# jacarvalho/mpd-public

Measured on AMD Instinct MI355X. Metric: denoising-steps/s, higher is better.
Workload: dtype f32; 1 GPU; cfg2: EnvDense2D-RobotPointMass shape, 100 trajectories (1 context(s)) x H=64 x D=4, T=100 (+5) reverse steps, unguided, U-Net dim_mults (1, 2, 4, 8), one plan = one bench step; parallelism=single, denoising_steps_per_plan=105

## Files before the change

### include/mpdx.h

```cpp
#ifndef MPDX_H
#define MPDX_H

#include <stddef.h>
#include <stdint.h>

#ifdef __cplusplus
extern "C" {
#endif

#define MPDX_E_INVALID   (-1)
#define MPDX_E_NOTFOUND  (-2)
#define MPDX_E_STATE     (-3)

#define MPDX_MAX_LEVELS 8

typedef struct mpdx_unet mpdx_unet;

typedef struct mpdx_unet_cfg {
    int32_t state_dim;
    int32_t n_support_points;
    int32_t unet_input_dim;
    int32_t n_levels;
    int32_t dim_mults[MPDX_MAX_LEVELS];
    int32_t time_emb_dim;
    int32_t self_attention;
} mpdx_unet_cfg;

const char* mpdx_last_error(void);
int mpdx_version(void);

int    mpdx_unet_create(const mpdx_unet_cfg* cfg, mpdx_unet** out);
void   mpdx_unet_destroy(mpdx_unet* u);
int    mpdx_unet_set_plan_join(mpdx_unet* u, int on);
int    mpdx_unet_plan_joined(const mpdx_unet* u);
int    mpdx_unet_num_params(const mpdx_unet* u);
int    mpdx_unet_param_info(const mpdx_unet* u, int idx, const char** name, int32_t shape[3], int32_t* ndim);
size_t mpdx_unet_packed_floats(const mpdx_unet* u);
size_t mpdx_unet_timetab_floats(const mpdx_unet* u, int T);
size_t mpdx_unet_workspace_floats(const mpdx_unet* u, int B);
int    mpdx_unet_pack_param(mpdx_unet* u, const char* name, const float* src_dev, size_t n_floats,
                            float* packed_dev, void* stream);
int    mpdx_unet_build_timetab(mpdx_unet* u, const float* packed_dev, const float* freqs16_dev, int T,
                               float* timetab_dev, void* stream);

int mpdx_unet_forward(mpdx_unet* u, const float* packed_dev, const float* timetab_dev, int T,
                      const float* x, int t, float* eps, int B, float* ws, void* stream);

typedef struct mpdx_step_coefs {
    float sqrt_recip_alphas_cumprod;
// ... 198 lines not shown
```

### mpd_public_amd/_lib.py

```python
from __future__ import annotations

import ctypes as C
from pathlib import Path

import os as _os

_LIB_PATH = Path(_os.environ["MPDX_LIB"]) if _os.environ.get("MPDX_LIB") else Path(__file__).resolve().parent / "libmpdx.so"
_lib = None

MAX_LEVELS = 8


class UnetCfg(C.Structure):
    _fields_ = [("state_dim", C.c_int32), ("n_support_points", C.c_int32), ("unet_input_dim", C.c_int32),
                ("n_levels", C.c_int32), ("dim_mults", C.c_int32 * MAX_LEVELS), ("time_emb_dim", C.c_int32),
                ("self_attention", C.c_int32)]


class StepCoefs(C.Structure):
    _fields_ = [("sqrt_recip_alphas_cumprod", C.c_float), ("sqrt_recipm1_alphas_cumprod", C.c_float),
                ("posterior_mean_coef1", C.c_float), ("posterior_mean_coef2", C.c_float),
                ("noise_scale", C.c_float), ("noise_std_extra", C.c_float),
                ("predict_epsilon", C.c_int32), ("clip_denoised", C.c_int32), ("ddim_k1", C.c_float), ("ddim_k2", C.c_float),
                ("guide_scale", C.c_float)]
# ... 41 lines not shown

class IkOpts(C.Structure):
    _fields_ = [("frame", C.c_int32), ("offset", C.c_float * 3), ("q_lo", C.c_float * 8), ("q_hi", C.c_float * 8), ("rot_weight", C.c_float),
                ("pos_tol", C.c_float), ("rot_tol", C.c_float), ("lambda_init", C.c_float), ("lambda_up", C.c_float), ("lambda_down", C.c_float),
                ("lambda_min", C.c_float), ("lambda_max", C.c_float), ("adaptive", C.c_int32), ("max_iters", C.c_int32), ("seed", C.c_uint64)]


_vp, _sz, _i, _f = C.c_void_p, C.c_size_t, C.c_int, C.c_float
SIGNATURES = {
    "mpdx_last_error": (C.c_char_p, []),
    "mpdx_version": (_i, []),
    "mpdx_unet_create": (_i, [C.POINTER(UnetCfg), C.POINTER(_vp)]),
    "mpdx_unet_destroy": (None, [_vp]),
    "mpdx_unet_set_plan_join": (_i, [_vp, _i]),
    "mpdx_unet_plan_joined": (_i, [_vp]),
    "mpdx_unet_num_params": (_i, [_vp]),
    "mpdx_unet_param_info": (_i, [_vp, _i, C.POINTER(C.c_char_p), C.POINTER(C.c_int32 * 3), C.POINTER(C.c_int32)]),
    "mpdx_unet_packed_floats": (_sz, [_vp]),
    "mpdx_unet_timetab_floats": (_sz, [_vp, _i]),
    "mpdx_unet_workspace_floats": (_sz, [_vp, _i]),
    "mpdx_unet_pack_param": (_i, [_vp, C.c_char_p, _vp, _sz, _vp, _vp]),
    "mpdx_unet_build_timetab": (_i, [_vp, _vp, _vp, _i, _vp, _vp]),
    "mpdx_unet_forward": (_i, [_vp, _vp, _vp, _i, _vp, _i, _vp, _i, _vp, _vp]),
    "mpdx_ddpm_step": (_i, [_vp, _vp, _vp, _i, _vp, _vp, _vp, _vp, C.POINTER(StepCoefs), _i, _i, _vp, _vp, _i, _i, _vp, _vp]),
    "mpdx_add_noise": (_i, [_vp, _vp, _vp, _vp, _f, _f, _vp, _i, _i, _i, _vp]),
    "mpdx_hard_conds": (_i, [_vp, _vp, _i, C.POINTER(C.c_int32), C.POINTER(_vp), _i, _i, _i, _vp]),
    "mpdx_q_sample": (_i, [_vp, _vp, _vp, _vp, _vp, _vp, _vp, _vp, _i, _i, _i, _i, _vp]),
    "mpdx_weighted_loss": (_i, [_vp, _vp, _vp, _vp, _vp, _i, _vp, _i, _i, _i, _vp]),
    "mpdx_plan": (_i, [_vp, _vp, _vp, _i, C.POINTER(StepCoefs), _i, _vp, _vp, _vp, _vp, _vp, _i, _vp,
                        C.POINTER(GuideParams), _i, _i, _vp, _i, C.c_uint64, C.c_uint64, _vp]),
# ... 83 lines not shown
```

### mpd_public_amd/csrc/conv_block.hpp

```cpp
#pragma once
#include <hip/hip_runtime.h>
#include <stdint.h>

#include <type_traits>

#if defined(MPDX_LOOP_ABLATION) && !defined(MPDX_DEV_HOOKS)
#define MPDX_DEV_HOOKS 1
#endif
#ifdef MPDX_DEV_HOOKS
#define MPDX_TRACE_PTR(p) (p)
#define MPDX_DBG(a, bits) ((a).dbg & (bits))
#else
#define MPDX_TRACE_PTR(p) ((long long*)nullptr)
#define MPDX_DBG(a, bits) (0)
#endif

namespace mpdx {

typedef float f32x4 __attribute__((ext_vector_type(4)));
typedef float f32x2 __attribute__((ext_vector_type(2)));

enum : int { CONV_S1 = 0, CONV_DOWN = 1, CONV_UPT = 2 };
enum : int { EPI_BIAS = 0, EPI_GN_MISH = 1, EPI_GN_MISH_GEN = 2, EPI_GN_BWD = 3 };

// ... 127 lines not shown

template <int MODE, int KS>
struct ConvGeom {
    static constexpr int PAD = (MODE == CONV_S1) ? KS / 2 : 1;
    static constexpr int NTAP = (MODE == CONV_UPT) ? 2 : KS;
    static constexpr int NSLOT = (MODE == CONV_UPT) ? 4 : KS;
};

__host__ __device__ inline int upt_slot_to_k(int slot) { return slot == 0 ? 1 : slot == 1 ? 3 : slot == 2 ? 2 : 0; }

struct GeoAny { static constexpr int L = 0, NC16 = 0, RSPAD = 0; };
template <int NC16_> struct GeoL8 { static constexpr int L = 8, NC16 = NC16_, RSPAD = 8; };
template <int NC16_> struct GeoUp8 { static constexpr int L = 8, NC16 = NC16_, RSPAD = 4; };
constexpr int geo_ilog2(int v) { return v <= 1 ? 0 : 1 + geo_ilog2(v >> 1); }

template <int MODE, int KS, int EPI, int MT, int NT, int WN, int WK, class GEO = GeoAny, int TBRES = -1>
__device__ __forceinline__ void conv_block_body(const ConvArgs& a, const int block_id) {
    using G = ConvGeom<MODE, KS>;
    constexpr bool GK = GEO::L > 0;
    static_assert(!GK || MODE == CONV_S1 || MODE == CONV_UPT, "compile-time geometry: stride-1 and transposed convolutions on 8 input positions");
    constexpr int NWAVE = WN * WK, NTHR = 64 * NWAVE;
    constexpr int MS = MT / 16, NSUB = NT / 16, NSW = NSUB / WN;
    constexpr int PAD = G::PAD, NTAP = G::NTAP, NSLOT = G::NSLOT;
    constexpr int MTP = MT + 4;
    constexpr int MTP4 = MTP / 4;
    static_assert(NSUB % WN == 0, "N split");
    static_assert(MODE != CONV_UPT || (NSW % 2 == 0), "transposed conv pairs even/odd sub-tiles");

    extern __shared__ __attribute__((aligned(16))) float smem[];

    const int tid = threadIdx.x, lane = tid & 63;
    if constexpr (GK) __builtin_assume(tid < NTHR);
// ... 33 lines not shown
#pragma unroll
            for (int p = 0; p < NCLS; ++p) {
                const int slot = (MODE == CONV_UPT) ? (p * 2 + ts) : ts;
                dst[m][p] = __builtin_bit_cast(f32x4, __builtin_amdgcn_raw_buffer_load_b128(wrs, wlane, wtile + ((m * nc16 + c16) * NSLOT + slot) * 1024, 0));
            }
    };
    const int niter = (ngroups + WK - 1) / WK;
    auto ring_g = [&](int it) { const int g = wk + it * WK; return g < ngroups ? g : ngroups - 1; };
    auto ring_init = [&]() {
#pragma unroll
        for (int u = 0; u < PF; ++u) load_a(ring_g(u), af[u]);
    };
#ifdef MPDX_RING_FIRST
    ring_init();
#endif

    if (!MPDX_DBG(a, 1)) {
        const int total = (spt << lg_Lin) << lg_c4n;
        const bool vec_ok = GK ? true : ((a.c1 & 3) == 0) && ((a.c2 & 3) == 0);
        constexpr int SB = 4;
        auto stage_pass = [&](int base, auto vec, auto first) {
            constexpr bool VEC = decltype(vec)::value;
            constexpr bool FIRST = decltype(first)::value;
            f32x4 v[SB];
            int dsto[SB], cc[SB];
            bool ok[SB];
            size_t pos[SB];
#pragma unroll
            for (int u = 0; u < SB; ++u) {
                const int idx = base + u * NTHR;
                const bool in = idx < total;
                const int idc = in ? idx : 0;
                const int rowi = idc >> lg_c4n, c = (idc & (c4n - 1)) << 2;
                const int s = rowi >> lg_Lin, li = rowi & (L_in - 1);
                const int b = s0 + s;
                dsto[u] = in ? (s * LP + li + PAD) * RS4 + (c >> 2) : -1;
                ok[u] = in && b < a.B && c < cin;
                cc[u] = c < cin ? c : 0;
                pos[u] = (size_t)(b < a.B ? b : a.B - 1) * L_in + li;
                if (a.stuff) { ok[u] = ok[u] && !(li & 1); pos[u] = (size_t)(b < a.B ? b : a.B - 1) * (L_in >> 1) + (li >> 1); }
            }
#pragma unroll
            for (int u = 0; u < SB; ++u) {
                if constexpr (VEC) {
                    const float* src = (cc[u] < a.c1) ? a.src1 + pos[u] * a.c1 + cc[u] : a.src2 + pos[u] * a.c2 + (cc[u] - a.c1);
                    v[u] = *(const f32x4*)src;
                } else {
#pragma unroll
                    for (int e = 0; e < 4; ++e) {
                        const int ce = cc[u] + e;
                        const float* src = (ce < a.c1) ? a.src1 + pos[u] * a.c1 + ce : (ce < cin) ? a.src2 + pos[u] * a.c2 + (ce - a.c1) : a.src1 + pos[u] * a.c1;
                        v[u][e] = *src;
                    }
                }
            }
#ifndef MPDX_RING_FIRST
            if constexpr (FIRST) ring_init();
#endif
#pragma unroll
            for (int u = 0; u < SB; ++u) {
                if constexpr (!VEC) {
#pragma unroll
                    for (int e = 0; e < 4; ++e) v[u][e] = (cc[u] + e < cin) ? v[u][e] : 0.f;
                }
                if (dsto[u] >= 0) smem4[dsto[u]] = ok[u] ? v[u] : (f32x4){0.f, 0.f, 0.f, 0.f};
            }
        };
        if (vec_ok) {
            stage_pass(tid, std::true_type{}, std::true_type{});
            for (int base = tid + NTHR * SB; base < total; base += NTHR * SB) stage_pass(base, std::true_type{}, std::false_type{});
        } else {
            stage_pass(tid, std::false_type{}, std::true_type{});
            for (int base = tid + NTHR * SB; base < total; base += NTHR * SB) stage_pass(base, std::false_type{}, std::false_type{});
        }
        if (PAD > 0) {
            constexpr int P2 = PAD > 0 ? 2 * PAD : 1;
            const int htot = (spt * P2) << lg_c4n;
            for (int idx = tid; idx < htot; idx += NTHR) {
                const int hr = idx >> lg_c4n, c4 = idx & (c4n - 1);
                const int s = hr / P2, k = hr - s * P2;
                const int lp = (k < PAD) ? k : (L_in + k);
                smem4[(s * LP + lp) * RS4 + c4] = (f32x4){0.f, 0.f, 0.f, 0.f};
            }
        }
    }
#ifndef MPDX_RING_FIRST
    if (MPDX_DBG(a, 1)) ring_init();
#endif
    CB_STAMP();
    __syncthreads();
    CB_STAMP();

    const int j = lane & 15, q = lane >> 4;
    int boff[NSW];
    int npos[NSW];
#pragma unroll
    for (int i = 0; i < NSW; ++i) {
        const int ns = wn * NSW + i;
        if (MODE == CONV_UPT) {
            const int gm = (ns >> 1) * 16 + j;
            const int s = gm >> lg_Lin, m = gm & (L_in - 1);
            boff[i] = (s * LP + m + PAD) * RS4 + q;
// ... 58 lines not shown

    CB_STAMP();
    __syncthreads();
    CB_STAMP();
    float* red = smem;
#pragma unroll
    for (int m = 0; m < MS; ++m)
#pragma unroll
        for (int i = 0; i < NSW; ++i)
            smem4[(wk * NT + npos[i]) * MTP4 + m * 4 + q] = acc[m][i];
    __syncthreads();
    CB_STAMP();

    if (MPDX_DBG(a, 4)) {
        if (tid == 0 && red[0] == 123.456f) a.dst[0] = red[1];
        return;
    }
    if constexpr (EPI == EPI_GN_MISH_GEN) {
        const int gs = a.gs;
        const int lg_gpt = (MT == 32 ? 5 : 4) - a.lg_gs;
        const int gpt = 1 << lg_gpt;
        const int nreg = spt << lg_gpt;
        const int re = gs << a.lg_Lout;
        const int Lv = (a.Lv_out > 0 && a.Lv_out < L_out) ? a.Lv_out : L_out;
        const float inv_re = 1.0f / (float)(gs * Lv);
        auto region = [&](auto w_, auto nch_, int s, int gl, int b) {
            constexpr int W = decltype(w_)::value, NCH = decltype(nch_)::value;
            float v[NCH][W], tb[NCH][W], rsd[NCH][W], ga[NCH][W], be[NCH][W];
            size_t o[NCH];
            bool ok[NCH];
            float sum = 0.f;
// ... 140 lines not shown
            if (re == 256) region(std::integral_constant<int, 4>{}, s, gl, s0 + s);
            else region(std::integral_constant<int, 2>{}, s, gl, s0 + s);
        }
    } else
    if (EPI == EPI_GN_MISH) {
        const int gs = a.gs;
        const int lg_gpt = (MT == 32 ? 5 : 4) - a.lg_gs;
        const int gpt = 1 << lg_gpt;
        const int nreg = spt << lg_gpt;
        const int re = gs << lg_Lout;
        const bool has_tb = TBRES < 0 ? a.tbias != nullptr : TBRES == 1, has_res = TBRES < 0 ? a.res != nullptr : TBRES == 2;
        const float inv_re = (re == 256) ? (1.0f / 256.0f) : (1.0f / 128.0f);
        for (int r = wave; r < nreg; r += NWAVE) {
            const int s = r >> lg_gpt, gl = r & (gpt - 1);
            const int b = s0 + s;
            if (re == 256) {
                const int e0 = lane * 4;
                const int l = e0 >> a.lg_gs, c = gl * gs + (e0 & (gs - 1));
                const int n = s * L_out + l, co = mt * MT + c;
                const size_t o = ((size_t)(b < a.B ? b : 0) * L_out + l) * a.C_out + co;
                const f32x4 bi = *(const f32x4*)(a.bias + co);
                const f32x4 ga = *(const f32x4*)(a.gamma + co), be = *(const f32x4*)(a.beta + co);
                f32x4 tb = {0.f, 0.f, 0.f, 0.f}, rs4 = {0.f, 0.f, 0.f, 0.f};
                if (has_tb) tb = *(const f32x4*)(a.tbias + (size_t)(b < a.B ? b : 0) * a.tb_stride + co);
                if (has_res) rs4 = *(const f32x4*)(a.res + o);
                const int ri = n * MTP4 + (c >> 2);
                f32x4 v = smem4[ri];
#pragma unroll
                for (int k = 1; k < WK; ++k) v += smem4[ri + k * NT * MTP4];
                v += bi;
// ... 50 lines not shown
            int ld = a.C_out, cc = co;
            if (a.c_split > 0) {
                if (co >= a.c_split) { d = a.dst2; cc = co - a.c_split; ld = a.C_out - a.c_split; }
                else ld = a.c_split;
            }
            if (a.decim && (l & 1)) continue;
            if (b < a.B && d) {
                f32x4* q = a.decim ? (f32x4*)(d + ((size_t)b * (L_out >> 1) + (l >> 1)) * ld + cc) : (f32x4*)(d + ((size_t)b * L_out + l) * ld + cc);
                if (a.accum & (d == a.dst2 ? 2 : 1)) v += *q;
                if (a.Lv_out > 0 && l >= a.Lv_out) v = (f32x4){0.f, 0.f, 0.f, 0.f};
                *q = v;
            }
        }
    }
    CB_STAMP();
#undef CB_STAMP
}

template <int MODE, int KS, int EPI, int MT, int NT, int WN, int WK, class GEO = GeoAny, int TBRES = -1>
__global__ __launch_bounds__(64 * WN * WK) void conv_block_kernel(const ConvArgs a) {
    conv_block_body<MODE, KS, EPI, MT, NT, WN, WK, GEO, TBRES>(a, blockIdx.x);
}

template <int MT, int NT, class GEO = GeoAny>
__global__ __launch_bounds__(512) void conv_pair_kernel(const ConvArgs a1, const ConvArgs a2, const int n_first) {
    if ((int)blockIdx.x < n_first) conv_block_body<CONV_S1, 5, EPI_GN_MISH, MT, NT, 1, 8, GEO, (GEO::L > 0 ? 1 : -1)>(a1, blockIdx.x);
    else conv_block_body<CONV_S1, 1, EPI_BIAS, MT, NT, 1, 8, GEO>(a2, blockIdx.x - n_first);
}

template <int MODE, int KS, int MT, int NT, int WK>
inline size_t conv_block_lds_bytes(int L_in, int L_out, int rs) {
// ... 8 lines not shown
```

### mpd_public_amd/csrc/host.hpp

```cpp
#pragma once
#include <hip/hip_runtime.h>

#include <algorithm>
#include <cmath>
#include <cstdarg>
#include <cstdio>
#include <cstdlib>
#include <cstring>
#include <mutex>
#include <set>
#include <string>
#include <unordered_map>
#include <vector>

#include "../../include/mpdx.h"
#include "conv_block.hpp"
#include "conv_ws.hpp"
#include "fused_level.hpp"
#include "switches.hpp"
#include "train_types.hpp"

namespace mpdx {

int fail(int code, const char* fmt, ...);
// ... 61 lines not shown
    mpdx_unet_cfg cfg;
    std::vector<mpdx::Param> params;
    std::unordered_map<std::string, int> pidx;
    std::vector<mpdx::Layer> layers;
    size_t packed_floats = 0;
    size_t slot_floats = 0;
    int n_slots = 0;
    int tt_row = 0;
    std::vector<int> tt_w, tt_b, tt_cout, tt_off;
    int final_slot = 0;
    int n_done = 0;
    int Hc = 0, xpad_slot = -1;
    bool masked() const { return Hc != cfg.n_support_points; }
    int plan_joined = 0;
    int plan_join = 1;
    struct CopyJob { size_t src, dst; int n0, ss0, ds0, n1, ss1, ds1, n_inner; };
    struct Fused {
        int first = 0, count = 0;
        bool has_final = false;
        int in1 = 0, in2 = 0;
        int in3 = mpdx::SRC_NONE;
        int gout_slot[3] = {-1, -1, -1};
        size_t lds_bytes = 0;
        mpdx::FusedArgs tmpl;
        int program = -1;
        std::vector<CopyJob> jobs;
        std::vector<int> op_layer;
        int in3_consumer = -1;
    };
    std::vector<Fused> fused;
// ... 20 lines not shown

namespace mpdx {

int pick_row_stride(int cin_pad, int mode, int L_in, int L_out, int LP);
void choose_tile(const Layer& l, int B, int& MT, int& NT);
bool layer_ksplit(const Layer& l);
int check_ready(const mpdx_unet* u);
unsigned fused_mask(int B);
bool fused_save_variant(const mpdx_unet::Fused& f);
int ensure_fused_streams(mpdx_unet* u, const float* packed, hipStream_t st);
int claim_fused_stream_jobs(mpdx_unet* u, const float* packed, const void** jobs, int* n);
int launch_final_step(const FinalArgs& fa, hipStream_t st);
int launch_conv_layer(const Layer& l, ConvArgs& a, int B, hipStream_t st);
bool pair_tile(const Layer& l1, const Layer& l2, int B, int& MT, int& NT);
int launch_conv_pair(int MT, int NT, const ConvArgs& a1, const ConvArgs& a2, const Layer& l1, const Layer& l2, hipStream_t st);
struct AttnArgs;
const char* attn_unsupported(int C, int L);
int launch_attention(const Layer& l, AttnArgs& a, int B, hipStream_t st);
int launch_weight_stationary(int variant, const Layer& l, ConvArgs& a, const ConvArgs& a2, int B, hipStream_t st);
int launch_fused_args(const mpdx_unet::Fused& f, const FusedArgs& a, int B, hipStream_t st, bool save = false);
int launch_fused_train(const mpdx_unet::Fused& f, const FusedArgs& a, int B, hipStream_t st);
int launch_fused_join(const FusedJoinArgs& ja, int B, hipStream_t st);
size_t fused_join_lds_bytes();
struct NoiseRng;
int launch_guide(const mpdx_guide_params* gp, float* x, float* grad_out, const float* hs, const float* hg, const uint32_t* amax_in,
                 uint32_t* amax_out, int n_per_ctx, int B, int H, int D, hipStream_t st, const float* noise = nullptr, float noise_scale = 0.f,
                 float noise_extra = 0.f, float* chain = nullptr, float guide_scale = 1.0f, const NoiseRng* rng = nullptr);
const char* chain_params_problem(const mpdx_guide_params& gp);
struct ChainInfo;
int guide_block_problem(const mpdx_guide_params* gp, int D, ChainInfo* chain_info);
// ... 3 lines not shown
```

### mpd_public_amd/csrc/mpdx.hip

```cpp
#include "host.hpp"
#include "attn.hpp"
#include "loss.hpp"
#include "scene_table.hpp"

namespace mpdx {

static thread_local char g_err[512] = "";
int fail(int code, const char* fmt, ...) {
    va_list ap;
    va_start(ap, fmt);
    vsnprintf(g_err, sizeof(g_err), fmt, ap);
    va_end(ap);
    return code;
}

int raise_lds_limit(const void* kern) {
    static std::mutex mu;
    static std::set<std::pair<int, const void*>> done;
    int dev = 0;
    HIP_TRY(hipGetDevice(&dev));
    std::lock_guard<std::mutex> lock(mu);
    if (done.count({dev, kern})) return 0;
    HIP_TRY(hipFuncSetAttribute(kern, hipFuncAttributeMaxDynamicSharedMemorySize, 160 * 1024));
    done.insert({dev, kern});
// ... 777 lines not shown
                              float* ws, FinalArgs& fa, hipStream_t st) {
    if (int rc = check_ready(u)) return rc;
    if (t < 0 || t >= T) return fail(MPDX_E_INVALID, "timestep %d outside [0,%d)", t, T);
    if (B <= 0) return fail(MPDX_E_INVALID, "B must be positive");
    const float* row = timetab + (size_t)t * u->tt_row;
    if (u->masked()) {
        float* xc = ws + u->slot_floats * (size_t)B * u->xpad_slot;
        const size_t nx = (size_t)B * u->Hc * u->cfg.state_dim;
        hipLaunchKernelGGL(pad_input_kernel, dim3((unsigned)std::min<size_t>((nx + 255) / 256, 2048)), dim3(256), 0, st, x, xc, B, u->cfg.n_support_points, u->Hc,
                           u->cfg.state_dim);
        x = xc;
    }
    return walk_pass(u, current_units(u, B, nullptr), packed, row, x, ws, B, fa, st, [](PassEvent, int) { return 0; });
}

static int run_plan_pass(mpdx_unet* u, const float* packed, const float* timetab, int T, const float* x, int t, int B, float* ws, FinalArgs& fa,
                         hipStream_t st, bool skip_down, const float* tt_next) {
    if (!skip_down && !tt_next) return run_unet_and_final(u, packed, timetab, T, x, t, B, ws, fa, st);
    const float* row = timetab + (size_t)t * u->tt_row;
    const auto units = current_units(u, B, nullptr);
    const int n = (int)units.size();
    for (int i = skip_down ? 1 : 0; i < n - (tt_next ? 1 : 0); ++i)
        if (int rc = run_unit(u, units[i], packed, row, x, ws, B, &fa, st)) return rc;
    if (tt_next) return run_fused_join(u, u->fused[units[n - 1].fused], u->fused[units[0].fused], packed, row, tt_next, x, ws, B, &fa, st);
    return 0;
}
static bool can_join_passes(const mpdx_unet* u, int B) {
    if (!u->plan_join || u->masked()) return false;
    const auto units = current_units(u, B, nullptr);
    if (units.size() < 2 || units.front().fused < 0 || units.back().fused < 0 || units.front().fused == units.back().fused) return false;
    const mpdx_unet::Fused& dn = u->fused[units.front().fused];
    const mpdx_unet::Fused& up = u->fused[units.back().fused];
    if (dn.program != 5 || dn.in1 != SRC_X || dn.in2 != SRC_NONE || dn.has_final || up.program != 3 || !up.has_final) return false;
    int dev = 0, cus = 0;
    if (hipGetDevice(&dev) != hipSuccess || hipDeviceGetAttribute(&cus, hipDeviceAttributeMultiprocessorCount, dev) != hipSuccess) return false;
    return B <= cus;
}

int dev_hooks_missing(const char* fn) {
// ... 51 lines not shown
            }
    if ((int)u->tt_w.size() > 40) { delete u; return fail(MPDX_E_INVALID, "too many residual blocks"); }
    build_units(u);
    u->packed_floats += 64;
    *out = u;
    return 0;
}

int mpdx_unet_set_plan_join(mpdx_unet* u, int on) {
    if (!u) return fail(MPDX_E_INVALID, "null argument");
    u->plan_join = on ? 1 : 0;
    return 0;
}
int mpdx_unet_plan_joined(const mpdx_unet* u) { return u ? u->plan_joined : 0; }

void mpdx_unet_destroy(mpdx_unet* u) {
    if (u && u->pack_descs_dev) (void)hipFree(u->pack_descs_dev);
    if (u && u->pack_chunks_dev) (void)hipFree(u->pack_chunks_dev);
    if (u && u->jobs_dev) (void)hipFree(u->jobs_dev);
    delete u;
}

int mpdx_unet_num_params(const mpdx_unet* u) { return u ? (int)u->params.size() : 0; }

int mpdx_unet_param_info(const mpdx_unet* u, int idx, const char** name, int32_t shape[3], int32_t* ndim) {
    if (!u || idx < 0 || idx >= (int)u->params.size()) return fail(MPDX_E_INVALID, "bad parameter index %d", idx);
    const Param& p = u->params[idx];
    if (name) *name = p.name.c_str();
    if (shape) { shape[0] = p.shape[0]; shape[1] = p.shape[1]; shape[2] = p.shape[2]; }
    if (ndim) *ndim = p.ndim;
    return 0;
}

size_t mpdx_unet_packed_floats(const mpdx_unet* u) { return u ? u->packed_floats : 0; }
// ... 115 lines not shown
int mpdx_weighted_loss(const float* pred, const float* targ, const float* weights_hd, const float* hard_start, const float* hard_goal,
                       int l1, float* out1, int B, int H, int D, void* stream) {
    if (!pred || !targ || !out1 || B <= 0) return fail(MPDX_E_INVALID, "bad argument");
    hipLaunchKernelGGL(weighted_loss_kernel, dim3(1), dim3(1024), 0, (hipStream_t)stream, pred, targ, weights_hd, hard_start, hard_goal, l1, out1,
                       B, H, D);
    HIP_TRY(hipGetLastError());
    return 0;
}

int mpdx_plan(mpdx_unet* u, const float* packed, const float* timetab, int T, const mpdx_step_coefs* coefs, int n_without_noise,
              float* x, const float* noise, const float* hard_start, const float* hard_goal, float* chain, int B, float* ws,
              const mpdx_guide_params* guide, int n_guide_steps, int t_start_guide, uint32_t* guide_flags, int n_per_ctx,
              uint64_t rng_seed, uint64_t rng_offset, void* stream) {
    if (!u || !packed || !timetab || !coefs || !x || !ws || T <= 0 || n_without_noise < 0 || B <= 0)
        return fail(MPDX_E_INVALID, "bad argument");
    if (guide)
        if (const char* why = scene_params_problem(*guide)) return fail(MPDX_E_INVALID, "%s", why);
    if (guide)
        if (const char* why = chain_params_problem(*guide)) return fail(MPDX_E_INVALID, "%s", why);
    if (int rc = check_ready(u)) return rc;
    hipStream_t st = (hipStream_t)stream;
    const int H = u->cfg.n_support_points, D = u->cfg.state_dim;
    const size_t n = (size_t)B * H * D;
    const int npc = n_per_ctx > 0 ? n_per_ctx : B;
    const int n_ctx = (B + npc - 1) / npc;
    const int steps = T + n_without_noise;
    if (n_guide_steps < 0) return fail(MPDX_E_INVALID, "n_guide_steps %d", n_guide_steps);
    if (n_guide_steps == 0) guide = nullptr;
    const int dbg = sw::debug();
    if (guide) {
        if (!guide_flags) return fail(MPDX_E_INVALID, "guide needs guide_flags");
        if (B % npc) return fail(MPDX_E_INVALID, "B=%d is not a multiple of n_per_ctx=%d", B, npc);
        HIP_TRY(hipMemsetAsync(guide_flags, 0, (size_t)steps * (n_guide_steps + 1) * n_ctx * sizeof(uint32_t), st));
    }
    hipLaunchKernelGGL(add_noise_kernel, dim3((unsigned)std::min<size_t>((n + 255) / 256, 2048)), dim3(256), 0, st, x, (const float*)nullptr,
                       hard_start, hard_goal, 0.f, 0.f, chain, B, H, D);
    const bool join_ok = can_join_passes(u, B);
    bool down_done = false;
    u->plan_joined = 0;
    int k = 0;
    for (int i = T - 1; i >= -n_without_noise; --i, ++k) {
        const int t = i < 0 ? 0 : i;
        const bool guided = guide && i < t_start_guide;
        const bool join = join_ok && !guided && i > -n_without_noise;
        const float* tt_next = join ? timetab + (size_t)(i - 1 < 0 ? 0 : i - 1) * u->tt_row : nullptr;
        const float* nz = (t == 0 || !noise) ? nullptr : noise + (size_t)k * n;
        NoiseRng rng;
        memset(&rng, 0, sizeof(rng));
        if (!noise && t != 0) { rng.on = 1; rng.seed = rng_seed; rng.offset = rng_offset; rng.elem0 = (unsigned long long)(k + 1) * n; }
        float* ch = chain ? chain + (size_t)(k + 1) * n : nullptr;
        uint32_t* fl = guided ? guide_flags + (size_t)k * (n_guide_steps + 1) * n_ctx : nullptr;
        FinalArgs fa;
        memset(&fa, 0, sizeof(fa));
        fa.x_in = x; fa.out = x;
        fa.k = coefs[t];
        fa.n_per_ctx = npc;
        if (!guided) {
            fa.rng = rng; fa.noise = nz; fa.hs = hard_start; fa.hg = hard_goal;
            fa.chain = ch; fa.mode = 1;
        } else {
            fa.mode = 2; fa.absmax = fl;
        }
        if (int rc = run_plan_pass(u, packed, timetab, T, x, t, B, ws, fa, st, down_done, tt_next)) return rc;
        down_done = join;
        u->plan_joined += join ? 1 : 0;
        if (guided) {
            for (int j = 0; j < n_guide_steps; ++j) {
                const bool last = j == n_guide_steps - 1;
                if (int rc = launch_guide(guide, x, nullptr, hard_start, hard_goal, fl + (size_t)j * n_ctx, fl + (size_t)(j + 1) * n_ctx, npc, B, H,
                                          D, st, last ? nz : nullptr, coefs[t].noise_scale, coefs[t].noise_std_extra, last ? ch : nullptr,
                                          coefs[t].guide_scale, last ? &rng : nullptr))
                    return rc;
            }
        }
        if (dbg) {
            if (dbg >= 2) {
                const hipError_t e = hipStreamSynchronize(st);
                if (e != hipSuccess) return fail((int)e, "mpdx_plan: loop iteration %d (t=%d%s) faulted: %s", k, t, guided ? ", guided" : "", hipGetErrorString(e));
            }
            hipError_t e = hipGetLastError();
            if (e != hipSuccess) return fail((int)e, "mpdx_plan: launch in loop iteration %d (t=%d%s) failed: %s", k, t, guided ? ", guided" : "", hipGetErrorString(e));
        }
    }
    HIP_TRY(hipGetLastError());
    return 0;
}

int mpdx_randn(float* out, size_t n, uint64_t seed, uint64_t offset, void* stream) {
    if (!out) return fail(MPDX_E_INVALID, "null argument");
    if (n == 0) return 0;
    const size_t nquad = (n + 3) / 4;
    hipLaunchKernelGGL(randn_kernel, dim3((unsigned)std::min<size_t>((nquad + 255) / 256, 4096)), dim3(256), 0, (hipStream_t)stream, out, n,
                       seed, offset);
    HIP_TRY(hipGetLastError());
    return 0;
}

int mpdx_attention_block(float* x, const float* to_qkv_w, const float* to_out_w, const float* to_out_b, const float* norm_g, const float* norm_b,
                         int B, int L, int Lv, int C, void* stream) {
    if (!x || !to_qkv_w || !to_out_w || !to_out_b || !norm_g || !norm_b) return fail(MPDX_E_INVALID, "null argument");
// ... 34 lines not shown
```

### mpd_public_amd/temporal_unet.py

```python
from __future__ import annotations

import ctypes as C
import math

import torch
import torch.nn as nn

from . import _lib

UNET_DIM_MULTS = {0: (1, 2, 4), 1: (1, 2, 4, 8)}


def group_norm_n_groups(n_channels, target_n_groups=8):
    if n_channels < target_n_groups:
        return 1
    for n_groups in range(target_n_groups, target_n_groups + 10):
        if n_channels % n_groups == 0:
            return n_groups
    return 1


class _Holder(nn.Module):

    def forward(self, *a, **k):
# ... 120 lines not shown
        if self._h is None:
            lib = _lib.load()
            mults = (C.c_int32 * _lib.MAX_LEVELS)(*self.dim_mults)
            cfg = _lib.UnetCfg(int(self.state_dim), int(self.n_support_points), int(self.unet_input_dim), len(self.dim_mults),
                               mults, int(self.time_emb_dim), int(self.self_attention))
            h = C.c_void_p()
            _lib.check(lib.mpdx_unet_create(C.byref(cfg), C.byref(h)), "mpdx_unet_create")
            self._h = h
        return self._h

    def set_plan_join(self, on: bool):
        _lib.check(_lib.load().mpdx_unet_set_plan_join(self._handle(), int(bool(on))), "mpdx_unet_set_plan_join")

    def plan_joined(self) -> int:
        return int(_lib.load().mpdx_unet_plan_joined(self._handle()))

    def _param_stamp(self):
        d = self.__dict__
        n = d.get("_stamp_calls", 0) + 1
        d["_stamp_calls"] = n
        pl = d.get("_plist")
        if pl is None or n % 16 == 0:
            pl = d["_plist"] = list(self.parameters())
        return tuple((p.data_ptr(), p._version) for p in pl)

    def _apply(self, fn, *a, **k):
        self.__dict__["_plist"] = None
        return super()._apply(fn, *a, **k)

    def load_state_dict(self, *a, **k):
# ... 69 lines not shown
```

Measured before the change: 5965 denoising-steps/s.

## Fuse seven innermost-level GroupNorm conv layers into one persistent kernel with counter sync

Adds an inner-run kernel that executes seven consecutive 256-channel, 8-position stride-1 conv+GroupNorm+Mish layers in a single launch. Per-cluster workgroups synchronise between layers with global atomic counters and a bounded spin wait, so the per-layer kernel launches and gaps at the bottleneck level go away. If a wait exceeds its budget, the kernel writes NaNs and sets a host-mapped status word. The change adds a dependency on co-residency of the workgroups and extra per-layer padding and zeroing setup. It is enabled by default for the 4-level, H=64 configuration.

```diff
diff --git a/include/mpdx.h b/include/mpdx.h
--- a/include/mpdx.h
+++ b/include/mpdx.h
@@ -11,6 +11,7 @@
 #define MPDX_E_INVALID   (-1)
 #define MPDX_E_NOTFOUND  (-2)
 #define MPDX_E_STATE     (-3)
+#define MPDX_E_DEVICE    (-4)
 
 #define MPDX_MAX_LEVELS 8
 
@@ -33,6 +34,10 @@
 void   mpdx_unet_destroy(mpdx_unet* u);
 int    mpdx_unet_set_plan_join(mpdx_unet* u, int on);
 int    mpdx_unet_plan_joined(const mpdx_unet* u);
+int    mpdx_unet_set_inner_run(mpdx_unet* u, int on);
+int    mpdx_unet_inner_runs(const mpdx_unet* u);
+int    mpdx_unet_status(const mpdx_unet* u);
+int    mpdx_unet_set_status(mpdx_unet* u, unsigned word);
 int    mpdx_unet_num_params(const mpdx_unet* u);
 int    mpdx_unet_param_info(const mpdx_unet* u, int idx, const char** name, int32_t shape[3], int32_t* ndim);
 size_t mpdx_unet_packed_floats(const mpdx_unet* u);
diff --git a/mpd_public_amd/_lib.py b/mpd_public_amd/_lib.py
--- a/mpd_public_amd/_lib.py
+++ b/mpd_public_amd/_lib.py
@@ -79,6 +79,10 @@
     "mpdx_unet_destroy": (None, [_vp]),
     "mpdx_unet_set_plan_join": (_i, [_vp, _i]),
     "mpdx_unet_plan_joined": (_i, [_vp]),
+    "mpdx_unet_set_inner_run": (_i, [_vp, _i]),
+    "mpdx_unet_inner_runs": (_i, [_vp]),
+    "mpdx_unet_status": (_i, [_vp]),
+    "mpdx_unet_set_status": (_i, [_vp, C.c_uint]),
     "mpdx_unet_num_params": (_i, [_vp]),
     "mpdx_unet_param_info": (_i, [_vp, _i, C.POINTER(C.c_char_p), C.POINTER(C.c_int32 * 3), C.POINTER(C.c_int32)]),
     "mpdx_unet_packed_floats": (_sz, [_vp]),
diff --git a/mpd_public_amd/csrc/conv_block.hpp b/mpd_public_amd/csrc/conv_block.hpp
--- a/mpd_public_amd/csrc/conv_block.hpp
+++ b/mpd_public_amd/csrc/conv_block.hpp
@@ -165,8 +165,19 @@
 template <int NC16_> struct GeoUp8 { static constexpr int L = 8, NC16 = NC16_, RSPAD = 4; };
 constexpr int geo_ilog2(int v) { return v <= 1 ? 0 : 1 + geo_ilog2(v >> 1); }
 
-template <int MODE, int KS, int EPI, int MT, int NT, int WN, int WK, class GEO = GeoAny, int TBRES = -1>
-__device__ __forceinline__ void conv_block_body(const ConvArgs& a, const int block_id) {
+struct RunCtx {
+    unsigned* counter = nullptr;
+    unsigned target = 0;
+    int wait = 0;
+    long long budget = 0;
+};
+constexpr unsigned kRunPoison = 0x10000000u;
+constexpr unsigned kRunPoisonSeen = 0x08000000u;
+
+typedef unsigned u32x4 __attribute__((ext_vector_type(4)));
+
+template <int MODE, int KS, int EPI, int MT, int NT, int WN, int WK, class GEO = GeoAny, int TBRES = -1, bool RUN = false>
+__device__ __forceinline__ bool conv_block_body(const ConvArgs& a, const int block_id, const RunCtx rc = RunCtx()) {
     using G = ConvGeom<MODE, KS>;
     constexpr bool GK = GEO::L > 0;
     static_assert(!GK || MODE == CONV_S1 || MODE == CONV_UPT, "compile-time geometry: stride-1 and transposed convolutions on 8 input positions");
@@ -230,6 +241,46 @@
 #ifdef MPDX_RING_FIRST
     ring_init();
 #endif
+    f32x4 run_bi = {0.f, 0.f, 0.f, 0.f}, run_ga = run_bi, run_be = run_bi, run_tb = run_bi;
+    if constexpr (RUN) {
+        static_assert(GK && MODE == CONV_S1 && EPI == EPI_GN_MISH && TBRES < 0 && WN == 1, "a run layer: stride-1 GroupNorm block with compile-time geometry");
+#ifndef MPDX_RING_FIRST
+        ring_init();
+#endif
+        const int co = mt * MT + ((lane * 4) & (MT - 1));
+        run_bi = *(const f32x4*)(a.bias + co);
+        run_ga = *(const f32x4*)(a.gamma + co); run_be = *(const f32x4*)(a.beta + co);
+        run_tb = *(const f32x4*)((a.tbias ? a.tbias : a.bias) + co);
+        {
+            constexpr int P2 = 2 * PAD;
+            const int htot = (spt * P2) << lg_c4n;
+            for (int idx = tid; idx < htot; idx += NTHR) {
+                const int hr = idx >> lg_c4n, c4 = idx & (c4n - 1);
+                const int s = hr / P2, k = hr - s * P2;
+                const int lp = (k < PAD) ? k : (L_in + k);
+                smem4[(s * LP + lp) * RS4 + c4] = (f32x4){0.f, 0.f, 0.f, 0.f};
+            }
+        }
+        CB_STAMP();
+        if (rc.wait) {
+            int* const flag = (int*)(smem + (GEO::NC16 * 16 + GEO::RSPAD) * (NT / GEO::L) * (GEO::L + 2 * PAD));
+            if (wave == 0) {
+                const long long t0 = (long long)__builtin_amdgcn_s_memtime();
+                int ok;
+                for (;;) {
+                    const unsigned v = __hip_atomic_load(rc.counter, __ATOMIC_RELAXED, __HIP_MEMORY_SCOPE_AGENT);
+                    const int d = (int)(v - rc.target);
+                    if (d >= 0) { ok = (unsigned)d < kRunPoisonSeen; break; }
+                    if ((long long)__builtin_amdgcn_s_memtime() - t0 > rc.budget) { ok = 0; break; }
+                    __builtin_amdgcn_s_sleep(1);
+                }
+                if (lane == 0) *flag = ok;
+            }
+            __syncthreads();
+            if (!*flag) return false;
+        }
+        CB_STAMP();
+    }
 
     if (!MPDX_DBG(a, 1)) {
         const int total = (spt << lg_Lin) << lg_c4n;
@@ -258,7 +309,10 @@
             }
 #pragma unroll
             for (int u = 0; u < SB; ++u) {
-                if constexpr (VEC) {
+                if constexpr (RUN) {
+                    const __amdgpu_buffer_rsrc_t srs = __builtin_amdgcn_make_buffer_rsrc((void*)a.src1, 0, 0x7fffffff, 0x00020000);
+                    v[u] = __builtin_bit_cast(f32x4, __builtin_amdgcn_raw_buffer_load_b128(srs, (int)(pos[u] * (GEO::NC16 * 16) + cc[u]) * 4, 0, 16));
+                } else if constexpr (VEC) {
                     const float* src = (cc[u] < a.c1) ? a.src1 + pos[u] * a.c1 + cc[u] : a.src2 + pos[u] * a.c2 + (cc[u] - a.c1);
                     v[u] = *(const f32x4*)src;
                 } else {
@@ -271,7 +325,7 @@
                 }
             }
 #ifndef MPDX_RING_FIRST
-            if constexpr (FIRST) ring_init();
+            if constexpr (FIRST && !RUN) ring_init();
 #endif
 #pragma unroll
             for (int u = 0; u < SB; ++u) {
@@ -289,7 +343,7 @@
             stage_pass(tid, std::false_type{}, std::true_type{});
             for (int base = tid + NTHR * SB; base < total; base += NTHR * SB) stage_pass(base, std::false_type{}, std::false_type{});
         }
-        if (PAD > 0) {
+        if (PAD > 0 && !RUN) {
             constexpr int P2 = PAD > 0 ? 2 * PAD : 1;
             const int htot = (spt * P2) << lg_c4n;
             for (int idx = tid; idx < htot; idx += NTHR) {
@@ -301,7 +355,7 @@
         }
     }
 #ifndef MPDX_RING_FIRST
-    if (MPDX_DBG(a, 1)) ring_init();
+    if (!RUN && MPDX_DBG(a, 1)) ring_init();
 #endif
     CB_STAMP();
     __syncthreads();
@@ -390,7 +444,7 @@
 
     if (MPDX_DBG(a, 4)) {
         if (tid == 0 && red[0] == 123.456f) a.dst[0] = red[1];
-        return;
+        return true;
     }
     if constexpr (EPI == EPI_GN_MISH_GEN) {
         const int gs = a.gs;
@@ -561,6 +615,32 @@
         for (int r = wave; r < nreg; r += NWAVE) {
             const int s = r >> lg_gpt, gl = r & (gpt - 1);
             const int b = s0 + s;
+            if constexpr (RUN) {
+                const int e0 = lane * 4;
+                const int l = e0 >> a.lg_gs, c = gl * gs + (e0 & (gs - 1));
+                const int n = s * L_out + l, co = mt * MT + c;
+                const size_t o = ((size_t)(b < a.B ? b : 0) * L_out + l) * a.C_out + co;
+                const __amdgpu_buffer_rsrc_t rrs = __builtin_amdgcn_make_buffer_rsrc((void*)(a.res ? a.res : a.src1), 0, 0x7fffffff, 0x00020000);
+                const f32x4 rs4 = __builtin_bit_cast(f32x4, __builtin_amdgcn_raw_buffer_load_b128(rrs, (int)o * 4, 0, 16));
+                const f32x4 ex = has_tb ? run_tb : rs4;
+                const int ri = n * MTP4 + (c >> 2);
+                f32x4 v = smem4[ri];
+#pragma unroll
+                for (int k = 1; k < WK; ++k) v += smem4[ri + k * NT * MTP4];
+                v += run_bi;
+                const float mean = wave_sum((v[0] + v[1]) + (v[2] + v[3])) * inv_re;
+                const f32x4 d = v - mean;
+                const float var = wave_sum((d[0] * d[0] + d[1] * d[1]) + (d[2] * d[2] + d[3] * d[3])) * inv_re;
+                const float rstd = gn_rstd(var);
+                f32x4 y;
+#pragma unroll
+                for (int e = 0; e < 4; ++e) y[e] = mish_nosel(d[e] * rstd * run_ga[e] + run_be[e]);
+                y += ex;
+                if (b < a.B) {
+                    const __amdgpu_buffer_rsrc_t drs = __builtin_amdgcn_make_buffer_rsrc((void*)a.dst, 0, 0x7fffffff, 0x00020000);
+                    __builtin_amdgcn_raw_buffer_store_b128(__builtin_bit_cast(u32x4, y), drs, (int)o * 4, 0, 16);
+                }
+            } else
             if (re == 256) {
                 const int e0 = lane * 4;
                 const int l = e0 >> a.lg_gs, c = gl * gs + (e0 & (gs - 1));
@@ -641,7 +721,14 @@
         }
     }
     CB_STAMP();
+    if constexpr (RUN) {
+        asm volatile("s_waitcnt vmcnt(0)" ::: "memory");
+        __syncthreads();
+        if (tid == 0) __hip_atomic_fetch_add(rc.counter, 1u, __ATOMIC_RELAXED, __HIP_MEMORY_SCOPE_AGENT);
+        CB_STAMP();
+    }
 #undef CB_STAMP
+    return true;
 }
 
 template <int MODE, int KS, int EPI, int MT, int NT, int WN, int WK, class GEO = GeoAny, int TBRES = -1>
diff --git a/mpd_public_amd/csrc/host.hpp b/mpd_public_amd/csrc/host.hpp
--- a/mpd_public_amd/csrc/host.hpp
+++ b/mpd_public_amd/csrc/host.hpp
@@ -99,6 +99,18 @@
     bool masked() const { return Hc != cfg.n_support_points; }
     int plan_joined = 0;
     int plan_join = 1;
+    int inner_run = 1;
+    int inner_runs = 0;
+    int run_capacity = -1;
+    long long run_budget = 0;
+    unsigned* run_counters = nullptr;
+    unsigned run_base = 0;
+    int run_live = 1 << 30;
+    bool run_rezero = false;
+    unsigned* run_status = nullptr;
+    unsigned* run_status_dev = nullptr;
+    unsigned status_host = 0;
+    unsigned status_word() const { return run_status ? __atomic_load_n(run_status, __ATOMIC_RELAXED) : status_host; }
     struct CopyJob { size_t src, dst; int n0, ss0, ds0, n1, ss1, ds1, n_inner; };
     struct Fused {
         int first = 0, count = 0;
@@ -149,6 +161,10 @@
 int launch_conv_layer(const Layer& l, ConvArgs& a, int B, hipStream_t st);
 bool pair_tile(const Layer& l1, const Layer& l2, int B, int& MT, int& NT);
 int launch_conv_pair(int MT, int NT, const ConvArgs& a1, const ConvArgs& a2, const Layer& l1, const Layer& l2, hipStream_t st);
+struct InnerRunArgs;
+int inner_run_grid(int B);
+int inner_run_workgroups_per_cu();
+int launch_inner_run(const InnerRunArgs& ra, int B, hipStream_t st);
 struct AttnArgs;
 const char* attn_unsupported(int C, int L);
 int launch_attention(const Layer& l, AttnArgs& a, int B, hipStream_t st);
diff --git a/mpd_public_amd/csrc/inner_run.hpp b/mpd_public_amd/csrc/inner_run.hpp
--- /dev/null
+++ b/mpd_public_amd/csrc/inner_run.hpp
@@ -0,0 +1,54 @@
+#pragma once
+#include "conv_block.hpp"
+
+namespace mpdx {
+
+constexpr int kInnerRunLayers = 7;
+constexpr int kInnerRunCounterStride = 32;
+
+struct InnerRunArgs {
+    ConvArgs layer[kInnerRunLayers];
+    unsigned* counters;
+    unsigned* status;
+    long long budget;
+    unsigned base;
+    int n_layers;
+    int nc;
+};
+
+constexpr size_t kInnerRunLds = (size_t)4 * 12 * (256 + 8) * sizeof(float) + 16;
+
+template <bool SAME_XCD>
+__global__ __launch_bounds__(512) void inner_run_kernel(const InnerRunArgs ra) {
+    int c, m;
+    if constexpr (SAME_XCD) {
+        const int b = blockIdx.x, x = b & 7, r = b >> 3;
+        m = r & 7; c = (r >> 3) * 8 + x;
+        if (c >= ra.nc) return;
+    } else {
+        c = (int)blockIdx.x >> 3; m = blockIdx.x & 7;
+    }
+    warm_kernarg<sizeof(InnerRunArgs)>();
+    RunCtx rc;
+    rc.counter = ra.counters + (size_t)c * kInnerRunCounterStride;
+    rc.budget = ra.budget;
+#pragma nounroll
+    for (int i = 0; i < ra.n_layers; ++i) {
+        rc.wait = i > 0;
+        rc.target = ra.base + 8u * (unsigned)i;
+        if (conv_block_body<CONV_S1, 5, EPI_GN_MISH, 32, 32, 1, 8, GeoL8<16>, -1, true>(ra.layer[i], c * 8 + m, rc)) continue;
+        const int tid = threadIdx.x;
+        if (tid == 0) {
+            __hip_atomic_fetch_or(ra.status, 1u | ((unsigned)i << 8), __ATOMIC_RELAXED, __HIP_MEMORY_SCOPE_SYSTEM);
+            __hip_atomic_store(rc.counter, rc.target + kRunPoison, __ATOMIC_RELAXED, __HIP_MEMORY_SCOPE_AGENT);
+        }
+        const ConvArgs& last = ra.layer[ra.n_layers - 1];
+        for (int e = tid; e < 4 * 8 * 32; e += 512) {
+            const int b = c * 4 + (e >> 8), l = (e >> 5) & 7, ch = m * 32 + (e & 31);
+            if (b < last.B) last.dst[((size_t)b * 8 + l) * 256 + ch] = __builtin_nanf("");
+        }
+        return;
+    }
+}
+
+}
diff --git a/mpd_public_amd/csrc/k_inner_run.hip b/mpd_public_amd/csrc/k_inner_run.hip
--- /dev/null
+++ b/mpd_public_amd/csrc/k_inner_run.hip
@@ -0,0 +1,31 @@
+#include "host.hpp"
+#include "inner_run.hpp"
+
+namespace mpdx {
+
+#ifndef MPDX_INNER_RUN_SAME_XCD
+#define MPDX_INNER_RUN_SAME_XCD 1
+#endif
+static constexpr bool kSameXcd = MPDX_INNER_RUN_SAME_XCD != 0;
+
+int inner_run_grid(int B) {
+    const int nc = (B + 3) / 4;
+    return kSameXcd ? ((nc + 7) / 8) * 64 : nc * 8;
+}
+
+int inner_run_workgroups_per_cu() {
+    int n = 0;
+    if (hipOccupancyMaxActiveBlocksPerMultiprocessor(&n, (const void*)inner_run_kernel<kSameXcd>, 512, kInnerRunLds) != hipSuccess) {
+        (void)hipGetLastError();
+        return 0;
+    }
+    return n;
+}
+
+int launch_inner_run(const InnerRunArgs& ra, int B, hipStream_t st) {
+    if (ra.n_layers < 1 || ra.n_layers > kInnerRunLayers || ra.nc != (B + 3) / 4) return fail(MPDX_E_INVALID, "inner run: %d layers, %d clusters for B=%d", ra.n_layers, ra.nc, B);
+    hipLaunchKernelGGL(inner_run_kernel<kSameXcd>, dim3(inner_run_grid(B)), dim3(512), kInnerRunLds, st, ra);
+    return 0;
+}
+
+}
diff --git a/mpd_public_amd/csrc/mpdx.hip b/mpd_public_amd/csrc/mpdx.hip
--- a/mpd_public_amd/csrc/mpdx.hip
+++ b/mpd_public_amd/csrc/mpdx.hip
@@ -1,5 +1,6 @@
 #include "host.hpp"
 #include "attn.hpp"
+#include "inner_run.hpp"
 #include "loss.hpp"
 #include "scene_table.hpp"
 
@@ -815,15 +816,96 @@
     return walk_pass(u, current_units(u, B, nullptr), packed, row, x, ws, B, fa, st, [](PassEvent, int) { return 0; });
 }
 
+static int inner_run_first(const mpdx_unet* u, const std::vector<mpdx_unet::Unit>& units, int B) {
+    if (!u->inner_run || u->masked() || u->cfg.self_attention || u->cfg.n_levels != 4 || u->cfg.n_support_points != 64) return -1;
+    if (u->run_capacity <= 0 || inner_run_grid(B) > u->run_capacity || !sw::geo() || sw::debug()) return -1;
+    auto fits = [&](const mpdx_unet::Unit& un) {
+        if (un.fused >= 0 || un.pair) return false;
+        const Layer& l = u->layers[un.layer];
+        if (l.attn || !(l.mode == CONV_S1 && l.ks == 5 && l.epi == EPI_GN_MISH) || l.Lv_out) return false;
+        if (!(l.c1 == 256 && l.c2 == 0 && l.src2 == SRC_NONE && l.cout == 256 && l.L_in == 8 && l.L_out == 8 && l.gs == 32 && l.cin_pad == 256 && l.rs == 264)) return false;
+        if ((l.tb_off >= 0) == (l.res != SRC_NONE)) return false;
+        return layer_ksplit(l);
+    };
+    const int n = (int)units.size();
+    for (int i = 0; i + kInnerRunLayers <= n; ++i) {
+        int k = 0;
+        while (k < kInnerRunLayers && fits(units[i + k])) ++k;
+        if (k == kInnerRunLayers) return i;
+    }
+    return -1;
+}
+static int ensure_inner_run_state(mpdx_unet* u) {
+    if (u->run_capacity >= 0) return 0;
+    u->run_capacity = 0;
+    int dev = 0, cus = 0, khz = 0;
+    if (hipGetDevice(&dev) != hipSuccess || hipDeviceGetAttribute(&cus, hipDeviceAttributeMultiprocessorCount, dev) != hipSuccess ||
+        hipDeviceGetAttribute(&khz, hipDeviceAttributeClockRate, dev) != hipSuccess) {
+        (void)hipGetLastError();
+        return 0;
+    }
+    const int per_cu = inner_run_workgroups_per_cu();
+    if (per_cu <= 0 || cus <= 0) return 0;
+    const int cap = cus;
+    const size_t words = (size_t)((cap + 7) / 8 + 8) * kInnerRunCounterStride;
+    HIP_TRY(hipMalloc((void**)&u->run_counters, words * sizeof(unsigned)));
+    HIP_TRY(hipMemset(u->run_counters, 0, words * sizeof(unsigned)));
+    HIP_TRY(hipHostMalloc((void**)&u->run_status, 64, hipHostMallocMapped));
+    *u->run_status = u->status_host;
+    HIP_TRY(hipHostGetDevicePointer((void**)&u->run_status_dev, u->run_status, 0));
+    u->run_budget = 4LL * (khz > 0 ? khz : 2400000);
+    u->run_capacity = cap;
+    return 0;
+}
+static int handle_status_error(const mpdx_unet* u, const char* fn) {
+    const unsigned w = u->status_word();
+    if (!w) return 0;
+    return fail(MPDX_E_DEVICE, "%s: a workgroup of the inner-level run gave up its wait (status 0x%x: layer %u of the run); the outputs of that plan hold NaN. "
+                "mpdx_unet_set_status(u, 0) clears the word", fn, w, w >> 8);
+}
+static int run_inner_run(mpdx_unet* u, const std::vector<mpdx_unet::Unit>& units, int first, const float* packed, const float* row, const float* x,
+                         float* ws, int B, hipStream_t st) {
+    InnerRunArgs ra;
+    memset(&ra, 0, sizeof(ra));
+    for (int k = 0; k < kInnerRunLayers; ++k) {
+        if (int rc = make_conv_args(u, u->layers[units[first + k].layer], packed, row, x, ws, B, 0, ra.layer[k])) return rc;
+        ra.layer[k].n_tiles_n = (B + 3) / 4;
+        ra.layer[k].trace = nullptr;
+    }
+    const int nc = (B + 3) / 4;
+    if (u->run_rezero || nc > u->run_live) {
+        HIP_TRY(hipMemsetAsync(u->run_counters, 0, (size_t)((u->run_capacity + 7) / 8 + 8) * kInnerRunCounterStride * sizeof(unsigned), st));
+        u->run_base = 0; u->run_rezero = false;
+    }
+    u->run_live = nc;
+    ra.counters = u->run_counters; ra.status = u->run_status_dev; ra.budget = u->run_budget;
+    ra.base = u->run_base;
+    ra.n_layers = kInnerRunLayers; ra.nc = (B + 3) / 4;
+    u->run_base += 8u * kInnerRunLayers;
+    u->inner_runs++;
+    return launch_inner_run(ra, B, st);
+}
+
 static int run_plan_pass(mpdx_unet* u, const float* packed, const float* timetab, int T, const float* x, int t, int B, float* ws, FinalArgs& fa,
-                         hipStream_t st, bool skip_down, const float* tt_next) {
-    if (!skip_down && !tt_next) return run_unet_and_final(u, packed, timetab, T, x, t, B, ws, fa, st);
+                         hipStream_t st, bool skip_down, const float* tt_next, bool use_run) {
+    if (!skip_down && !tt_next && !use_run) return run_unet_and_final(u, packed, timetab, T, x, t, B, ws, fa, st);
+    if (t < 0 || t >= T) return fail(MPDX_E_INVALID, "timestep %d outside [0,%d)", t, T);
     const float* row = timetab + (size_t)t * u->tt_row;
     const auto units = current_units(u, B, nullptr);
     const int n = (int)units.size();
-    for (int i = skip_down ? 1 : 0; i < n - (tt_next ? 1 : 0); ++i)
+    const int rf = use_run ? inner_run_first(u, units, B) : -1;
+    bool final_done = false;
+    for (int i = skip_down ? 1 : 0; i < n - (tt_next ? 1 : 0); ++i) {
+        if (i == rf) {
+            if (int rc = run_inner_run(u, units, rf, packed, row, x, ws, B, st)) return rc;
+            i += kInnerRunLayers - 1;
+            continue;
+        }
+        if (units[i].fused >= 0) final_done |= u->fused[units[i].fused].has_final;
         if (int rc = run_unit(u, units[i], packed, row, x, ws, B, &fa, st)) return rc;
+    }
     if (tt_next) return run_fused_join(u, u->fused[units[n - 1].fused], u->fused[units[0].fused], packed, row, tt_next, x, ws, B, &fa, st);
+    if (!final_done) return run_final(u, packed, fa, B, ws, st);
     return 0;
 }
 static bool can_join_passes(const mpdx_unet* u, int B) {
@@ -905,10 +987,30 @@
 }
 int mpdx_unet_plan_joined(const mpdx_unet* u) { return u ? u->plan_joined : 0; }
 
+int mpdx_unet_set_inner_run(mpdx_unet* u, int on) {
+    if (!u) return fail(MPDX_E_INVALID, "null argument");
+    u->inner_run = on ? 1 : 0;
+    return 0;
+}
+int mpdx_unet_inner_runs(const mpdx_unet* u) { return u ? u->inner_runs : 0; }
+int mpdx_unet_status(const mpdx_unet* u) {
+    if (!u) return fail(MPDX_E_INVALID, "null argument");
+    return handle_status_error(u, "mpdx_unet_status");
+}
+int mpdx_unet_set_status(mpdx_unet* u, unsigned word) {
+    if (!u) return fail(MPDX_E_INVALID, "null argument");
+    if (u->run_status) __atomic_store_n(u->run_status, word, __ATOMIC_RELAXED);
+    u->status_host = word;
+    if (!word && u->run_counters) u->run_rezero = true;
+    return 0;
+}
+
 void mpdx_unet_destroy(mpdx_unet* u) {
     if (u && u->pack_descs_dev) (void)hipFree(u->pack_descs_dev);
     if (u && u->pack_chunks_dev) (void)hipFree(u->pack_chunks_dev);
     if (u && u->jobs_dev) (void)hipFree(u->jobs_dev);
+    if (u && u->run_counters) (void)hipFree(u->run_counters);
+    if (u && u->run_status) (void)hipHostFree(u->run_status);
     delete u;
 }
 
@@ -1054,6 +1156,7 @@
               uint64_t rng_seed, uint64_t rng_offset, void* stream) {
     if (!u || !packed || !timetab || !coefs || !x || !ws || T <= 0 || n_without_noise < 0 || B <= 0)
         return fail(MPDX_E_INVALID, "bad argument");
+    if (int rc = handle_status_error(u, "mpdx_plan")) return rc;
     if (guide)
         if (const char* why = scene_params_problem(*guide)) return fail(MPDX_E_INVALID, "%s", why);
     if (guide)
@@ -1076,6 +1179,12 @@
     hipLaunchKernelGGL(add_noise_kernel, dim3((unsigned)std::min<size_t>((n + 255) / 256, 2048)), dim3(256), 0, st, x, (const float*)nullptr,
                        hard_start, hard_goal, 0.f, 0.f, chain, B, H, D);
     const bool join_ok = can_join_passes(u, B);
+    u->inner_runs = 0;
+    bool use_run = false;
+    if (u->inner_run && !u->masked() && !u->cfg.self_attention && u->cfg.n_levels == 4 && H == 64) {
+        if (int rc = ensure_inner_run_state(u)) return rc;
+        use_run = inner_run_first(u, current_units(u, B, nullptr), B) >= 0;
+    }
     bool down_done = false;
     u->plan_joined = 0;
     int k = 0;
@@ -1101,7 +1210,7 @@
         } else {
             fa.mode = 2; fa.absmax = fl;
         }
-        if (int rc = run_plan_pass(u, packed, timetab, T, x, t, B, ws, fa, st, down_done, tt_next)) return rc;
+        if (int rc = run_plan_pass(u, packed, timetab, T, x, t, B, ws, fa, st, down_done, tt_next, use_run)) return rc;
         down_done = join;
         u->plan_joined += join ? 1 : 0;
         if (guided) {
@@ -1123,7 +1232,7 @@
         }
     }
     HIP_TRY(hipGetLastError());
-    return 0;
+    return use_run ? handle_status_error(u, "mpdx_plan") : 0;
 }
 
 int mpdx_randn(float* out, size_t n, uint64_t seed, uint64_t offset, void* stream) {
diff --git a/mpd_public_amd/temporal_unet.py b/mpd_public_amd/temporal_unet.py
--- a/mpd_public_amd/temporal_unet.py
+++ b/mpd_public_amd/temporal_unet.py
@@ -158,6 +158,15 @@
 
     def plan_joined(self) -> int:
         return int(_lib.load().mpdx_unet_plan_joined(self._handle()))
+
+    def set_inner_run(self, on: bool):
+        _lib.check(_lib.load().mpdx_unet_set_inner_run(self._handle(), int(bool(on))), "mpdx_unet_set_inner_run")
+
+    def inner_runs(self) -> int:
+        return int(_lib.load().mpdx_unet_inner_runs(self._handle()))
+
+    def status(self) -> int:
+        return int(_lib.load().mpdx_unet_status(self._handle()))
 
     def _param_stamp(self):
         d = self.__dict__
```

Measured after the change: 6268 denoising-steps/s (median of 6 runs). +5.1%, better.
